# traveller59/spconv

Measured on NVIDIA H100. Metric: active-voxels/sec fwd+bwd SubMConv3d 3^3 C=64, higher is better.
Workload: dtype fp16

## Files before the change

spconv_b200/csrc/common.cuh:

```cuda
#pragma once
#include <cuda_runtime.h>
#include <cuda_fp16.h>
#include <cuda_bf16.h>
#include <stdint.h>
#include <stdio.h>
#include <string.h>
#include <stdarg.h>
#include <type_traits>

#include "../../include/spconv_b200.h"

namespace spx {

void set_error(const char *fmt, ...);
void count_launch(int n = 1);
void set_family(int f);
int sm_count();
int current_device();

struct RuntimeCfg {
    int force_simt = 0, force_tc = 0;
    int debug = 0;
    long long *trace = nullptr;
};
// ... 61 lines not shown
template <typename T> __device__ __forceinline__ float to_float(T v);
template <> __device__ __forceinline__ float to_float<float>(float v) { return v; }
template <> __device__ __forceinline__ float to_float<__half>(__half v) { return __half2float(v); }
template <> __device__ __forceinline__ float to_float<__nv_bfloat16>(__nv_bfloat16 v) { return __bfloat162float(v); }
template <> __device__ __forceinline__ float to_float<int8_t>(int8_t v) { return (float)v; }

template <typename T> __device__ __forceinline__ T from_float(float v);
template <> __device__ __forceinline__ float from_float<float>(float v) { return v; }
template <> __device__ __forceinline__ __half from_float<__half>(float v) { return __float2half_rn(v); }
template <> __device__ __forceinline__ __nv_bfloat16 from_float<__nv_bfloat16>(float v) { return __float2bfloat16_rn(v); }

__device__ __forceinline__ float apply_act(float v, int act, float alpha) {
    switch (act) {
        case SPX_ACT_RELU: return v > 0.f ? v : 0.f;
        case SPX_ACT_SIGMOID: return 1.f / (1.f + __expf(-v));
        case SPX_ACT_LEAKY_RELU: return v >= 0.f ? v : v * alpha;
        default: return v;
    }
}

__device__ __forceinline__ uint32_t smem_u32(const void *p) {
    return (uint32_t)__cvta_generic_to_shared(p);
}

__device__ __forceinline__ void mbar_init(uint64_t *bar, uint32_t count) {
    asm volatile("mbarrier.init.shared::cta.b64 [%0], %1;" ::"r"(smem_u32(bar)), "r"(count) : "memory");
}
__device__ __forceinline__ void mbar_fence_init() {
    asm volatile("fence.mbarrier_init.release.cluster;" ::: "memory");
}
__device__ __forceinline__ void mbar_arrive(uint64_t *bar) {
    asm volatile("{\n\t.reg .b64 st;\n\tmbarrier.arrive.shared::cta.b64 st, [%0];\n\t}" ::"r"(smem_u32(bar)) : "memory");
}
__device__ __forceinline__ void mbar_arrive_expect_tx(uint64_t *bar, uint32_t bytes) {
    asm volatile("{\n\t.reg .b64 st;\n\tmbarrier.arrive.expect_tx.shared::cta.b64 st, [%0], %1;\n\t}" ::"r"(smem_u32(bar)), "r"(bytes) : "memory");
}
__device__ __forceinline__ bool mbar_try_wait(uint64_t *bar, uint32_t parity) {
    uint32_t ok;
    asm volatile(
        "{\n\t.reg .pred p;\n\t"
        "mbarrier.try_wait.parity.shared::cta.b64 p, [%1], %2;\n\t"
        "selp.u32 %0, 1, 0, p;\n\t}"
        : "=r"(ok) : "r"(smem_u32(bar)), "r"(parity) : "memory");
    return ok != 0;
}
__device__ __forceinline__ void mbar_wait(uint64_t *bar, uint32_t parity) {
    if (mbar_try_wait(bar, parity)) return;
    const long long t0 = clock64();
    uint32_t spins = 0;
    while (!mbar_try_wait(bar, parity)) {
        if ((++spins & 0x3FFFu) == 0u && clock64() - t0 > 4000000000ll) {
            printf("spconv_b200: mbarrier wait timed out (block %d thread %d bar 0x%x parity %u)\n",
                   (int)blockIdx.x, (int)threadIdx.x, smem_u32(bar), parity);
            __trap();
        }
    }
}
__device__ __forceinline__ void cp_async_mbar_arrive_noinc(uint64_t *bar) {
    asm volatile("cp.async.mbarrier.arrive.noinc.shared::cta.b64 [%0];" ::"r"(smem_u32(bar)) : "memory");
}

__device__ __forceinline__ void cp_async_16(uint32_t dst_smem, const void *src, uint32_t src_bytes) {
    asm volatile("cp.async.cg.shared.global [%0], [%1], 16, %2;" ::"r"(dst_smem), "l"(src), "r"(src_bytes) : "memory");
}
__device__ __forceinline__ void cp_async_commit() { asm volatile("cp.async.commit_group;" ::: "memory"); }
template <int N> __device__ __forceinline__ void cp_async_wait() {
    asm volatile("cp.async.wait_group %0;" ::"n"(N) : "memory");
}

__device__ __forceinline__ void fence_proxy_async_smem() {
    asm volatile("fence.proxy.async.shared::cta;" ::: "memory");
}

__device__ __forceinline__ void tma_load_2d(uint32_t dst_smem, const void *tmap, uint64_t *bar,
                                            int32_t c0, int32_t c1) {
    asm volatile(
        "cp.async.bulk.tensor.2d.shared::cta.global.tile.mbarrier::complete_tx::bytes [%0], [%1, {%3, %4}], [%2];"
        ::"r"(dst_smem), "l"(tmap), "r"(smem_u32(bar)), "r"(c0), "r"(c1) : "memory");
}
__device__ __forceinline__ void bulk_copy_g2s(uint32_t dst_smem, const void *src, uint32_t bytes, uint64_t *bar) {
    asm volatile("cp.async.bulk.shared::cluster.global.mbarrier::complete_tx::bytes [%0], [%1], %2, [%3];"
                 ::"r"(dst_smem), "l"(src), "r"(bytes), "r"(smem_u32(bar)) : "memory");
}
__device__ __forceinline__ void tma_prefetch_desc(const void *tmap) {
    asm volatile("prefetch.tensormap [%0];" ::"l"(tmap) : "memory");
}

enum MmaKind { KIND_F16 = 0, KIND_TF32 = 1, KIND_I8 = 2 };

__device__ __forceinline__ void wgmma_fence() { asm volatile("wgmma.fence.sync.aligned;" ::: "memory"); }
__device__ __forceinline__ void wgmma_commit() { asm volatile("wgmma.commit_group.sync.aligned;" ::: "memory"); }
template <int N> __device__ __forceinline__ void wgmma_wait() {
    asm volatile("wgmma.wait_group.sync.aligned %0;" ::"n"(N) : "memory");
}
template <typename T, int R> __device__ __forceinline__ void fence_regs(T (&d)[R]) {
#pragma unroll
    for (int i = 0; i < R; ++i) {
        if constexpr (sizeof(T) == 4 && std::is_floating_point<T>::value) asm volatile("" : "+f"(d[i])::"memory");
        else asm volatile("" : "+r"(d[i])::"memory");
    }
}

__host__ __device__ __forceinline__ uint64_t gmma_desc_hi(uint32_t lbo_bytes, uint32_t sbo_bytes, uint32_t swizzle_bytes) {
    const uint64_t layout = swizzle_bytes == 128 ? 1ull : (swizzle_bytes == 64 ? 2ull : 3ull);
    return ((uint64_t)((lbo_bytes >> 4) & 0x3FFF) << 16) | ((uint64_t)((sbo_bytes >> 4) & 0x3FFF) << 32) | (layout << 62);
}

__device__ __forceinline__ uint32_t swizzle_offset(uint32_t off, uint32_t swizzle_bytes) {
    uint32_t bits = swizzle_bytes == 128 ? 7u : (swizzle_bytes == 64 ? 3u : 1u);
    return off ^ (((off >> 7) & bits) << 4);
}

#endif

}
```

spconv_b200/csrc/gemm_tc.cu:

```cuda
#include "gemm.cuh"
#include "wgmma.cuh"
#include <cuda.h>
#include <atomic>
#include <mutex>
#include <stdlib.h>

namespace spx {

constexpr int TC_TILE_M = 128;
constexpr int TC_CONS_WARPS = 8;
constexpr int TC_PROD_WARPS = 2;
constexpr int TC_PROD_THREADS = TC_PROD_WARPS * 32;
constexpr int TC_TMA_WARP = TC_CONS_WARPS + TC_PROD_WARPS;
constexpr int TC_SCHED_WARP = TC_TMA_WARP + 1;
constexpr int TC_THREADS = 3 * 128;
constexpr int TC_INFO_DEPTH = 4;
constexpr int TC_INFO_READERS = TC_PROD_WARPS + TC_CONS_WARPS + 1;
constexpr int TC_MAX_STAGES = 8;
constexpr int TC_SMEM_BUDGET = 200 * 1024;

struct TcParams {
    const uint8_t *x;
    int xb;
    int span_b, b_subtiles, b_sub_bytes, b_bytes, b_mn_major, b_kstep16_mn;
// ... 124 lines not shown
    constexpr int SPAN_A = XB < 128 ? XB : 128;
    constexpr int LG_SPAN_A = SPAN_A == 128 ? 7 : (SPAN_A == 64 ? 6 : 5);
    constexpr int A_SUB_BYTES = TC_TILE_M * SPAN_A;
    constexpr int A_SUBTILES = XB / SPAN_A;
    constexpr int Q_A = SPAN_A / 32;
    constexpr int ROWS_PW = TC_TILE_M / TC_PROD_WARPS;
    constexpr int ITERS = ROWS_PW / RPI > 0 ? ROWS_PW / RPI : 1;
    static_assert(ROWS_PW * CPR >= 32, "a producer warp must cover at least one full cp.async instruction");

    extern __shared__ __align__(1024) uint8_t smem_raw[];
    TC_SPAN(0);
    const uint32_t raw_addr = smem_u32(smem_raw);
    const uint32_t pad = (1024u - (raw_addr & 1023u)) & 1023u;
    uint8_t *smem = smem_raw + pad;
    const uint32_t smem_base = raw_addr + pad;

    const uint32_t idx_off = (uint32_t)p.stages * p.stage_bytes;
    uint64_t *bars = reinterpret_cast<uint64_t *>(smem + idx_off + 2u * p.idx_bytes);
    uint64_t *full = bars;
    uint64_t *empty = bars + TC_MAX_STAGES;
    uint64_t *idx_full = bars + 2 * TC_MAX_STAGES;
    uint64_t *idx_empty = bars + 2 * TC_MAX_STAGES + 2;
    uint64_t *info_full = bars + 2 * TC_MAX_STAGES + 4;
    uint64_t *info_empty = bars + 2 * TC_MAX_STAGES + 4 + TC_INFO_DEPTH;
    int32_t *info = reinterpret_cast<int32_t *>(bars + 2 * TC_MAX_STAGES + 4 + 2 * TC_INFO_DEPTH);

    const int warp = threadIdx.x >> 5;
    const int lane = threadIdx.x & 31;
    const int64_t num_tiles = (p.rows + TC_TILE_M - 1) / TC_TILE_M;

    auto read_info = [&](int n, uint32_t (&tm)[4]) -> int {
        const int e = n & (TC_INFO_DEPTH - 1);
        mbar_wait(&info_full[e], (uint32_t)((n / TC_INFO_DEPTH) & 1));
        const volatile int32_t *r = info + e * 8;
        const int tile = r[0];
        tm[0] = (uint32_t)r[1]; tm[1] = (uint32_t)r[2]; tm[2] = (uint32_t)r[3]; tm[3] = (uint32_t)r[4];
        __syncwarp();
        if (lane == 0) mbar_arrive(&info_empty[e]);
        return tile;
    };

    if (threadIdx.x == 0) {
        for (int s = 0; s < p.stages; ++s) {
            mbar_init(&full[s], TC_PROD_THREADS + 1);
            mbar_init(&empty[s], TC_CONS_WARPS);
        }
        for (int a = 0; a < 2; ++a) {
            mbar_init(&idx_full[a], 1);
            mbar_init(&idx_empty[a], TC_PROD_WARPS);
        }
        for (int e = 0; e < TC_INFO_DEPTH; ++e) {
            mbar_init(&info_full[e], 1);
            mbar_init(&info_empty[e], TC_INFO_READERS);
        }
        mbar_fence_init();
        tma_prefetch_desc(&tmap_w);
    }
    __syncthreads();
    TC_SPAN(1);

    if (warp >= TC_CONS_WARPS && warp < TC_TMA_WARP) {
        const int pw = warp - TC_CONS_WARPS;
        const int r0 = lane >> LG_CPR;
        const uint32_t byte_in_row = (uint32_t)(lane & (CPR - 1)) << 4;
        const uint8_t *x_lane = p.x + byte_in_row;
        uint32_t dst_off[ITERS];
#pragma unroll
        for (int itc = 0; itc < ITERS; ++itc) {
            const uint32_t row_in_tile = (uint32_t)(pw * ROWS_PW + r0 + itc * RPI);
            const uint32_t sub = byte_in_row >> LG_SPAN_A;
            const uint32_t within = byte_in_row & (uint32_t)(SPAN_A - 1);
            dst_off[itc] = sub * (uint32_t)A_SUB_BYTES + swizzle_offset((row_in_tile << LG_SPAN_A) + within, SPAN_A);
        }
        int stage = 0; uint32_t phase = 0;
        for (int n = 0;; ++n) {
            uint32_t tm[4];
            if (read_info(n, tm) < 0) break;
            const int buf = n & 1;
            mbar_wait(&idx_full[buf], (uint32_t)((n >> 1) & 1));
            const int32_t *idx_lane = reinterpret_cast<const int32_t *>(smem + idx_off + (size_t)buf * p.idx_bytes) +
                                      pw * ROWS_PW + r0;
            BitIter it(tm);
            int k = it.next();
            int32_t ridx[ITERS];
            if (k >= 0) {
#pragma unroll
                for (int itc = 0; itc < ITERS; ++itc) ridx[itc] = idx_lane[k * 128 + itc * RPI];
            }
            while (k >= 0) {
                mbar_wait(&empty[stage], phase ^ 1u);
                const uint32_t a_stage = smem_base + (uint32_t)stage * p.stage_bytes;
                if (!(p.debug & 1)) {
#pragma unroll
                    for (int itc = 0; itc < ITERS; ++itc)
                        cp_async_16(a_stage + dst_off[itc], x_lane + (int64_t)max(ridx[itc], 0) * XB,
                                    ridx[itc] >= 0 ? 16u : 0u);
                }
                cp_async_mbar_arrive_noinc(&full[stage]);
                k = it.next();
                if (k >= 0) {
#pragma unroll
                    for (int itc = 0; itc < ITERS; ++itc) ridx[itc] = idx_lane[k * 128 + itc * RPI];
                }
                if (++stage == p.stages) { stage = 0; phase ^= 1u; }
            }
            __syncwarp();
            if (lane == 0) mbar_arrive(&idx_empty[buf]);
        }
    } else if (warp == TC_TMA_WARP) {
        int stage = 0; uint32_t phase = 0;
        for (int n = 0;; ++n) {
            uint32_t tm[4];
            if (read_info(n, tm) < 0) break;
            BitIter it(tm);
            for (int k = it.next(); k >= 0; k = it.next()) {
                mbar_wait(&empty[stage], phase ^ 1u);
                const int kw = p.reverse ? p.kv - 1 - k : k;
                const uint32_t b_stage = smem_base + (uint32_t)stage * p.stage_bytes + p.a_stage_bytes;
                if (p.b_transposed) {
                    const int i4s = p.c_in >> 2;
                    const float *wk = p.w + (int64_t)kw * p.c_in;
                    for (int q = lane; q < p.c_out * i4s; q += 32) {
                        const int o = q / i4s, i4 = (q - o * i4s) * 4;
                        const float4 v = __ldg(reinterpret_cast<const float4 *>(wk + (int64_t)o * p.kv * p.c_in + i4));
                        const uint32_t kb = (uint32_t)o * 4u;
                        const uint32_t sub = kb / (uint32_t)p.span_b, within = kb % (uint32_t)p.span_b;
                        const float vv[4] = {v.x, v.y, v.z, v.w};
#pragma unroll
                        for (int t = 0; t < 4; ++t) {
                            const uint32_t off = sub * (uint32_t)p.b_sub_bytes +
                                                 swizzle_offset((uint32_t)(i4 + t) * (uint32_t)p.span_b + within, (uint32_t)p.span_b);
                            asm volatile("st.shared.f32 [%0], %1;" ::"r"(b_stage + off), "f"(vv[t]) : "memory");
                        }
                    }
                    fence_proxy_async_smem();
                    __syncwarp();
                    if (lane == 0) mbar_arrive(&full[stage]);
                } else if (lane == 0) {
                    if (p.debug & 8) {
                        mbar_arrive(&full[stage]);
                    } else {
                        mbar_arrive_expect_tx(&full[stage], (uint32_t)p.b_bytes);
                        for (int sb = 0; sb < p.b_subtiles; ++sb)
                            tma_load_2d(b_stage + sb * p.b_sub_bytes, &tmap_w, &full[stage],
                                        kw * p.w_inner_elems + sb * p.span_b_elems, 0);
                    }
                }
                __syncwarp();
                if (++stage == p.stages) { stage = 0; phase ^= 1u; }
            }
        }
    } else if (warp == TC_SCHED_WARP) {
        const uint32_t blk_bytes = (uint32_t)(p.kv + 1) * 512u;
        for (int n = 0;; ++n) {
            const int b = n & 1, e = n & (TC_INFO_DEPTH - 1);
            mbar_wait(&idx_empty[b], (uint32_t)(((n >> 1) & 1) ^ 1));
            mbar_wait(&info_empty[e], (uint32_t)(((n / TC_INFO_DEPTH) & 1) ^ 1));
            int tile = -1;
            if (lane == 0) {
                const int ticket = atomicAdd(p.sched_state, 1);
                int4 r0 = make_int4(-1, 1, 0, 0), r1 = make_int4(0, 0, 0, 0);
                if ((int64_t)ticket < num_tiles) {
                    const int4 *rp = reinterpret_cast<const int4 *>(p.sched_rec + (int64_t)ticket * TT_REC_INTS);
                    r0 = __ldg(rp); r1 = __ldg(rp + 1);
                }
                tile = r0.x;
                int32_t *dst = info + e * 8;
                dst[0] = r0.x; dst[1] = r0.y; dst[2] = r0.z; dst[3] = r0.w; dst[4] = r1.x;
                if (tile >= 0) {
                    mbar_arrive_expect_tx(&idx_full[b], blk_bytes);
                    bulk_copy_g2s(smem_base + idx_off + (uint32_t)b * p.idx_bytes,
                                  p.tile_table + (int64_t)tile * (p.kv + 1) * 128, blk_bytes, &idx_full[b]);
                }
                mbar_arrive(&info_full[e]);
            }
            tile = __shfl_sync(0xffffffffu, tile, 0);
            if (tile < 0) break;
        }
        if (lane == 0) {
            __threadfence();
            const int done = atomicAdd(p.sched_state + 1, 1);
            if (done == (int)gridDim.x - 1) {
                p.sched_state[0] = 0;
                p.sched_state[1] = 0;
                __threadfence();
            }
        }
        __syncwarp();
    } else if (warp < TC_CONS_WARPS) {
        const int wg = warp >> 2;
        int stage = 0; uint32_t phase = 0;
        const uint64_t a_hi = gmma_desc_hi(16u, 8u * SPAN_A, SPAN_A);
        const uint64_t b_hi = p.b_mn_major ? gmma_desc_hi((uint32_t)p.b_sub_bytes, 8u * p.span_b, p.span_b)
                                           : gmma_desc_hi(16u, 8u * p.span_b, p.span_b);
        const uint32_t b_sub16 = (uint32_t)p.b_sub_bytes >> 4;
        Acc acc[N / 2];
        for (int local = 0;; ++local) {
            uint32_t tm[4];
            const int tile = read_info(local, tm);
            if (tile < 0) break;
#pragma unroll
            for (int i = 0; i < N / 2; ++i) acc[i] = (Acc)0;
            BitIter it(tm);
            for (int k = it.next(); k >= 0; k = it.next()) {
                mbar_wait(&full[stage], phase);
                fence_proxy_async_smem();
                const uint32_t a16 = (smem_base + (uint32_t)stage * p.stage_bytes + (uint32_t)(wg * 64 * SPAN_A)) >> 4;
                const uint32_t b16 = (smem_base + (uint32_t)stage * p.stage_bytes + (uint32_t)p.a_stage_bytes) >> 4;
                if (!(p.debug & 2)) {
                    fence_regs(acc);
                    wgmma_fence();
                    if (!p.b_mn_major) {
#pragma unroll
                        for (int sub = 0; sub < A_SUBTILES; ++sub) {
                            const uint32_t as = a16 + (uint32_t)sub * (uint32_t)(A_SUB_BYTES >> 4);
                            const uint32_t bs = b16 + (uint32_t)sub * b_sub16;
#pragma unroll
                            for (int jr = 0; jr < Q_A; ++jr)
                                mma_step<KIND, N>(acc, a_hi | (uint64_t)((as + 2u * jr) & 0x3FFFu),
                                                  b_hi | (uint64_t)((bs + 2u * jr) & 0x3FFFu), 0, p.ab_bf16);
                        }
                    } else {
#pragma unroll
                        for (int sub = 0; sub < A_SUBTILES; ++sub) {
                            const uint32_t as = a16 + (uint32_t)sub * (uint32_t)(A_SUB_BYTES >> 4);
#pragma unroll
                            for (int jr = 0; jr < Q_A; ++jr) {
                                const uint32_t j = (uint32_t)(sub * Q_A + jr);
                                mma_step<KIND, N>(acc, a_hi | (uint64_t)((as + 2u * jr) & 0x3FFFu),
                                                  b_hi | (uint64_t)((b16 + j * (uint32_t)p.b_kstep16_mn) & 0x3FFFu), 1,
                                                  p.ab_bf16);
                            }
                        }
                    }
                    wgmma_commit();
                    wgmma_wait<0>();
                    fence_regs(acc);
                }
                __syncwarp();
                if (lane == 0) mbar_arrive(&empty[stage]);
                if (++stage == p.stages) { stage = 0; phase ^= 1u; }
            }
            if (p.debug & 4) continue;
            const int64_t r_lo = (int64_t)tile * TC_TILE_M + wg * 64 + (warp & 3) * 16 + (lane >> 2);
            const int64_t r_hi = r_lo + 8;
            int64_t d_lo = -1, d_hi = -1;
            if (r_lo < p.rows) d_lo = p.argsort ? (int64_t)__ldg(p.argsort + r_lo) : r_lo;
            if (r_hi < p.rows) d_hi = p.argsort ? (int64_t)__ldg(p.argsort + r_hi) : r_hi;
            if constexpr (KIND == KIND_F16) {
                if (p.out_dtype == SPX_F16) epilogue_frag<SPX_F16, false, N>(p, acc, d_lo, d_hi, lane);
                else epilogue_frag<SPX_BF16, false, N>(p, acc, d_lo, d_hi, lane);
            } else if constexpr (KIND == KIND_TF32) {
                epilogue_frag<SPX_F32, false, N>(p, acc, d_lo, d_hi, lane);
            } else {
                if (p.out_dtype == SPX_I8) epilogue_frag<SPX_I8, true, N>(p, acc, d_lo, d_hi, lane);
                else if (p.out_dtype == SPX_F32) epilogue_frag<SPX_F32, true, N>(p, acc, d_lo, d_hi, lane);
                else epilogue_frag<SPX_F16, true, N>(p, acc, d_lo, d_hi, lane);
            }
        }
// ... 201 lines not shown
```

spconv_b200/csrc/gemm_tc_wgrad.cu:

```cuda
#include "gemm.cuh"
#include "peer.cuh"
#include "wgmma.cuh"
#include <stdlib.h>

namespace spx {

constexpr int WG_TILE = 128;
constexpr int WG_CONS_WARPS = 8;
constexpr int WG_PROD_WARPS = 2;
constexpr int WG_PROD_THREADS = WG_PROD_WARPS * 32;
constexpr int WG_SCHED_WARP = WG_CONS_WARPS + WG_PROD_WARPS;
constexpr int WG_THREADS = 3 * 128;
constexpr int WG_ACC_COLS = 256;
constexpr int WG_MAX_STAGES = 6;
constexpr int WG_SMEM_BUDGET = 200 * 1024;
constexpr int WG_SMEM_MAX = 224 * 1024;
constexpr int WG_MAX_IDX = 4;

struct WgParams {
    const uint8_t *x; int xb, span_x, lg_span_x, apo, apg, atom_elems;
    const uint8_t *d; int db, span_d, lg_span_d, lg_cpr_d;
    int n, ab_bf16;
    int groups_total, groups_per_pass;
    int stages, a_stage_bytes, b_buf_bytes, idx_bytes, idx_bufs;
    int64_t rows;
    const int32_t *tile_table;
    const uint32_t *tile_mask;
    const int32_t *sched_rec;
    int kv, words, c_in;
    float *partial; int64_t partial_stride;
    long long *dbg_ts;
    int debug;
};

__device__ __forceinline__ int slot_offset(int slot, int kv) {
    if (slot >= kv) return kv;
    return (slot & 1) ? kv - 1 - (slot >> 1) : (slot >> 1);
}

__device__ __forceinline__ uint32_t active_groups(const uint32_t (&tm)[4], const uint32_t *gmask, int ng, int words) {
    uint32_t act = 0;
    if (words == 1) {
        for (int gl = 0; gl < ng; ++gl) act |= (tm[0] & gmask[gl * 4]) ? 1u << gl : 0u;
        return act;
    }
    for (int gl = 0; gl < ng; ++gl) {
        const uint32_t hit = (tm[0] & gmask[gl * 4]) | (tm[1] & gmask[gl * 4 + 1]) | (tm[2] & gmask[gl * 4 + 2]) |
                             (tm[3] & gmask[gl * 4 + 3]);
        if (hit) act |= 1u << gl;
    }
    return act;
}

__device__ __forceinline__ int64_t wg_rec_index(int64_t i, int chunk, int chunks) {
    return i * chunks + ((i & 1) ? (chunks - 1 - chunk) : chunk);
}
__device__ __forceinline__ void wg_load_rec(const int32_t *__restrict__ rec, int64_t r, int64_t &tile, uint32_t (&m)[4]) {
    const int4 a = __ldg(reinterpret_cast<const int4 *>(rec + r * TT_REC_INTS));
    const int b = __ldg(rec + r * TT_REC_INTS + 4);
    tile = a.x; m[0] = (uint32_t)a.y; m[1] = (uint32_t)a.z; m[2] = (uint32_t)a.w; m[3] = (uint32_t)b;
}

__device__ __forceinline__ long long wg_global_ns() {
    long long t;
    asm volatile("mov.u64 %0, %%globaltimer;" : "=l"(t));
    return t;
}
#define WG_SPAN(i) do { if (p.dbg_ts && threadIdx.x == 0) { const int c_ = blockIdx.y * gridDim.x + blockIdx.x; if (c_ < 512) p.dbg_ts[2 * 2048 + c_ * 4 + (i)] = wg_global_ns(); } } while (0)

__device__ __forceinline__ uint32_t pick_word(const uint32_t (&m)[4], int w) {
    return w == 0 ? m[0] : (w == 1 ? m[1] : (w == 2 ? m[2] : m[3]));
}

__device__ __forceinline__ uint32_t kmajor_tf32_off(uint32_t row, uint32_t voxel, uint32_t rows) {
    return (voxel >> 5) * rows * 128u + swizzle_offset(row * 128u + ((voxel & 31u) << 2), 128u);
}
__device__ __forceinline__ void st_shared_f32x4_t(uint32_t base, uint32_t row0, uint32_t voxel, uint32_t rows, float4 v) {
    const float f[4] = {v.x, v.y, v.z, v.w};
#pragma unroll
    for (int t = 0; t < 4; ++t)
        asm volatile("st.shared.f32 [%0], %1;" ::"r"(base + kmajor_tf32_off(row0 + t, voxel, rows)), "f"(f[t]) : "memory");
}

template <int CPA, int CPD, bool TF32 = false>
__global__ void __launch_bounds__(WG_THREADS, 1)
tc_wgrad_kernel(const WgParams p) {
    constexpr int E = TF32 ? 4 : 2;
    constexpr int N = CPD * 16 / E;
    constexpr int G = WG_ACC_COLS / N < 16 ? WG_ACC_COLS / N : 16;
    constexpr int KSTEPS = WG_TILE * E / 32;
    constexpr int LG_CPA = CPA == 2 ? 1 : (CPA == 4 ? 2 : 3);
    constexpr int RPI = 32 / CPA;
    constexpr int LG_CPD = CPD == 2 ? 1 : (CPD == 4 ? 2 : (CPD == 8 ? 3 : (CPD == 16 ? 4 : 5)));
    constexpr int RPI_D = 32 / CPD;
    constexpr int DB = CPD * 16;
    constexpr int SPAN_D = DB < 128 ? DB : 128;
    constexpr int LG_SPAN_D = SPAN_D == 128 ? 7 : (SPAN_D == 64 ? 6 : 5);
    constexpr int SPAN_X = CPA * 16;
    constexpr int LG_SPAN_X = LG_CPA + 4;
    constexpr int ROWS_PW = WG_TILE / WG_PROD_WARPS;
    constexpr int ITERS = ROWS_PW / RPI > 0 ? ROWS_PW / RPI : 1;
    constexpr int ITERS_D = ROWS_PW / RPI_D;
    extern __shared__ __align__(1024) uint8_t smem_raw[];
    WG_SPAN(0);
    const uint32_t raw_addr = smem_u32(smem_raw);
    const uint32_t pad = (1024u - (raw_addr & 1023u)) & 1023u;
    uint8_t *smem = smem_raw + pad;
    const uint32_t smem_base = raw_addr + pad;
    const uint32_t b_base = smem_base;
    const uint32_t a_base = smem_base + 2u * p.b_buf_bytes;
    const uint32_t idx_off = 2u * p.b_buf_bytes + (uint32_t)p.stages * p.a_stage_bytes;
    uint64_t *bars = reinterpret_cast<uint64_t *>(smem + idx_off + (uint32_t)p.idx_bufs * p.idx_bytes);
    uint64_t *full_a = bars;
    uint64_t *empty_a = bars + WG_MAX_STAGES;
    uint64_t *full_b = bars + 2 * WG_MAX_STAGES;
    uint64_t *empty_b = bars + 2 * WG_MAX_STAGES + 2;
    uint64_t *idx_full = bars + 2 * WG_MAX_STAGES + 4;
    uint64_t *idx_empty = bars + 2 * WG_MAX_STAGES + 4 + WG_MAX_IDX;
    uint32_t *gmask = reinterpret_cast<uint32_t *>(bars + 2 * WG_MAX_STAGES + 4 + 2 * WG_MAX_IDX);
    uint32_t *slot_info = gmask + 32 * 4;

    const int warp = threadIdx.x >> 5;
    const int lane = threadIdx.x & 31;
    const int64_t num_tiles = (p.rows + WG_TILE - 1) / WG_TILE;
    const int chunk = blockIdx.x, chunks = gridDim.x;
    const int g_first = blockIdx.y, g_step = gridDim.y;
    const int ng = g_first < p.groups_total ? (p.groups_total - g_first + g_step - 1) / g_step : 0;

    if (threadIdx.x < 32) {
        const int g = g_first + (int)threadIdx.x * g_step;
        uint32_t m[4] = {0, 0, 0, 0};
        if ((int)threadIdx.x < ng) {
            for (int a = g * p.apg; a < (g + 1) * p.apg; ++a) {
                const int k = slot_offset(a / p.apo, p.kv);
                if (k < p.kv) m[k >> 5] |= 1u << (k & 31);
            }
        }
#pragma unroll
        for (int w = 0; w < 4; ++w) gmask[threadIdx.x * 4 + w] = m[w];
    }
    if (threadIdx.x == 0) {
        for (int s = 0; s < p.stages; ++s) { mbar_init(&full_a[s], WG_PROD_THREADS); mbar_init(&empty_a[s], WG_CONS_WARPS); }
        for (int b = 0; b < 2; ++b) { mbar_init(&full_b[b], WG_PROD_THREADS); mbar_init(&empty_b[b], WG_CONS_WARPS); }
        for (int b = 0; b < p.idx_bufs; ++b) { mbar_init(&idx_full[b], 1); mbar_init(&idx_empty[b], WG_PROD_WARPS); }
        mbar_fence_init();
    }
    __syncthreads();
    WG_SPAN(1);

    if (warp >= WG_CONS_WARPS && warp < WG_SCHED_WARP) {
        const int pw = warp - WG_CONS_WARPS;
        int stage = 0; uint32_t phase = 0;
        int64_t nb = 0;
        const int r0 = lane >> LG_CPA;
        const uint32_t chb = (uint32_t)(lane & (CPA - 1)) << 4;
        const uint8_t *x_lane = p.x + chb;
        uint32_t dst_off[ITERS];
#pragma unroll
        for (int itc = 0; itc < ITERS; ++itc)
            dst_off[itc] = swizzle_offset(((uint32_t)(pw * ROWS_PW + r0 + itc * RPI) << LG_SPAN_X) + chb, SPAN_X);
        const int lg_apo = p.apo == 1 ? 0 : (p.apo == 2 ? 1 : 2);
        const int rd0 = lane >> LG_CPD;
        const uint32_t chd = (uint32_t)(lane & (CPD - 1)) << 4;
        const uint8_t *d_lane = p.d + chd;
        const int nring = p.idx_bufs;
        auto issue_b = [&](const int32_t *idx_s) {
            const int bb = (int)(nb & 1);
            mbar_wait(&empty_b[bb], (uint32_t)(((nb >> 1) & 1) ^ 1));
            const uint32_t dstb = b_base + (uint32_t)bb * p.b_buf_bytes;
            const int32_t *rows_s = idx_s + p.kv * 128 + pw * ROWS_PW + rd0;
            int32_t rsrc[ITERS_D];
#pragma unroll
            for (int itc = 0; itc < ITERS_D; ++itc) rsrc[itc] = rows_s[itc * RPI_D];
            if constexpr (TF32) {
#pragma unroll 1
                for (int i0 = 0; i0 < ITERS_D; i0 += 8) {
                    float4 v[8];
#pragma unroll
                    for (int i = 0; i < 8; ++i) {
                        const int32_t r = i0 + i < ITERS_D ? rsrc[i0 + i] : -1;
                        v[i] = r >= 0 ? __ldg(reinterpret_cast<const float4 *>(d_lane + (int64_t)r * DB)) : make_float4(0.f, 0.f, 0.f, 0.f);
                    }
#pragma unroll
                    for (int i = 0; i < 8; ++i)
                        if (i0 + i < ITERS_D)
                            st_shared_f32x4_t(dstb, chd >> 2, (uint32_t)(pw * ROWS_PW + rd0 + (i0 + i) * RPI_D), (uint32_t)N, v[i]);
                }
                fence_proxy_async_smem();
                mbar_arrive(&full_b[bb]);
            } else {
#pragma unroll
                for (int itc = 0; itc < ITERS_D; ++itc) {
                    const uint32_t row_in_tile = (uint32_t)(pw * ROWS_PW + rd0 + itc * RPI_D);
                    const uint32_t off = (chd >> LG_SPAN_D) * (uint32_t)(WG_TILE * SPAN_D) +
                                         swizzle_offset((row_in_tile << LG_SPAN_D) + (chd & (uint32_t)(SPAN_D - 1)), SPAN_D);
                    cp_async_16(dstb + off, d_lane + (int64_t)max(rsrc[itc], 0) * DB, rsrc[itc] >= 0 ? 16u : 0u);
                }
                cp_async_mbar_arrive_noinc(&full_b[bb]);
            }
            ++nb;
        };
        auto idx_block = [&](int b) {
            return reinterpret_cast<const int32_t *>(smem + idx_off + (size_t)b * p.idx_bytes);
        };
        auto read_slot = [&](int slot, uint32_t use, uint32_t (&m)[4]) -> uint32_t {
            mbar_wait(&idx_full[slot], use & 1u);
            const volatile uint32_t *r = slot_info + slot * 8;
            m[0] = r[1]; m[1] = r[2]; m[2] = r[3]; m[3] = r[4];
            return r[0];
        };
        int cur_slot = 0; uint32_t cur_use = 0;
        uint32_t tm[4] = {0, 0, 0, 0}, tm1[4] = {0, 0, 0, 0};
        uint32_t act = 0;
        if (wg_rec_index(0, chunk, chunks) < num_tiles) {
            act = read_slot(0, 0u, tm);
            if (act) issue_b(idx_block(0));
        }
        for (int64_t step = 0; wg_rec_index(step, chunk, chunks) < num_tiles; ++step) {
            const bool has_next = wg_rec_index(step + 1, chunk, chunks) < num_tiles;
            int nxt_slot = cur_slot + 1; uint32_t nxt_use = cur_use;
            if (nxt_slot == nring) { nxt_slot = 0; ++nxt_use; }
            uint32_t act_next = 0;
            bool next_ready = !has_next;
            auto prepare_next = [&]() {
                act_next = read_slot(nxt_slot, nxt_use, tm1);
                if (act_next) issue_b(idx_block(nxt_slot));
                next_ready = true;
            };
            const int32_t *idx_s = idx_block(cur_slot);
            for (uint32_t rem = act; rem; rem &= rem - 1) {
                const int g = g_first + (__ffs(rem) - 1) * g_step;
                mbar_wait(&empty_a[stage], phase ^ 1u);
                const uint32_t a_stage = a_base + (uint32_t)stage * p.a_stage_bytes;
                for (int s = 0; s < p.apg; ++s) {
                    const int a = g * p.apg + s;
                    const int k = slot_offset(a >> lg_apo, p.kv);
                    const int cb = a & (p.apo - 1);
                    const bool active = k < p.kv && ((pick_word(tm, k >> 5) >> (k & 31)) & 1u);
                    const int32_t *idx_k = idx_s + (active ? k : 0) * 128 + pw * ROWS_PW + r0;
                    const uint8_t *x_atom = x_lane + cb * SPAN_X;
                    int32_t ridx[ITERS];
#pragma unroll
                    for (int itc = 0; itc < ITERS; ++itc) ridx[itc] = active ? idx_k[itc * RPI] : -1;
                    if constexpr (TF32) {
#pragma unroll
                        for (int itc = 0; itc < ITERS; ++itc) {
                            float4 v = make_float4(0.f, 0.f, 0.f, 0.f);
                            if (ridx[itc] >= 0) v = __ldg(reinterpret_cast<const float4 *>(x_atom + (int64_t)ridx[itc] * p.xb));
                            st_shared_f32x4_t(a_stage, (uint32_t)(s * 32) + (chb >> 2),
                                              (uint32_t)(pw * ROWS_PW + r0 + itc * RPI), (uint32_t)WG_TILE, v);
                        }
                    } else {
                        const uint32_t atom_base = a_stage + (uint32_t)s * (uint32_t)(WG_TILE * SPAN_X);
#pragma unroll
                        for (int itc = 0; itc < ITERS; ++itc)
                            cp_async_16(atom_base + dst_off[itc], x_atom + (int64_t)max(ridx[itc], 0) * p.xb,
                                        ridx[itc] >= 0 ? 16u : 0u);
                    }
                }
                if constexpr (TF32) {
                    fence_proxy_async_smem();
                    mbar_arrive(&full_a[stage]);
                } else {
                    cp_async_mbar_arrive_noinc(&full_a[stage]);
                }
                if (++stage == p.stages) { stage = 0; phase ^= 1u; }
                if (!next_ready) prepare_next();
            }
            if (!next_ready) prepare_next();
            __syncwarp();
            if (lane == 0) mbar_arrive(&idx_empty[cur_slot]);
#pragma unroll
            for (int w = 0; w < 4; ++w) tm[w] = tm1[w];
            act = act_next;
            cur_slot = nxt_slot; cur_use = nxt_use;
        }
    } else if (warp == WG_SCHED_WARP) {
        const uint32_t blk_bytes = (uint32_t)(p.kv + 1) * 512u;
        const int nring = p.idx_bufs;
        int slot = 0; uint32_t use = 0;
        uint32_t mw[4] = {0, 0, 0, 0};
        int64_t mtile = 0;
        for (int64_t i = 0; wg_rec_index(i, chunk, chunks) < num_tiles; ++i) {
            if ((i & 31) == 0) {
                const int64_t r = wg_rec_index(i + lane, chunk, chunks);
                if (r < num_tiles) wg_load_rec(p.sched_rec, r, mtile, mw);
            }
            uint32_t tm[4];
#pragma unroll
            for (int w = 0; w < 4; ++w) tm[w] = __shfl_sync(0xffffffffu, mw[w], (int)(i & 31));
            const int64_t tile = __shfl_sync(0xffffffffu, mtile, (int)(i & 31));
            const uint32_t act = active_groups(tm, gmask, ng, p.words);
            mbar_wait(&idx_empty[slot], (use & 1u) ^ 1u);
            if (lane == 0) {
                uint32_t *r = slot_info + slot * 8;
                r[0] = act; r[1] = tm[0]; r[2] = tm[1]; r[3] = tm[2]; r[4] = tm[3];
                if (act) {
                    mbar_arrive_expect_tx(&idx_full[slot], blk_bytes);
                    bulk_copy_g2s(smem_base + idx_off + (uint32_t)slot * p.idx_bytes,
                                  p.tile_table + tile * (int64_t)(p.kv + 1) * 128, blk_bytes, &idx_full[slot]);
                } else {
                    mbar_arrive(&idx_full[slot]);
                }
            }
            __syncwarp();
            if (++slot == nring) { slot = 0; ++use; }
        }
    } else if (warp < WG_CONS_WARPS) {
        const int wg = warp >> 2;
        int stage = 0; uint32_t phase = 0;
        int64_t nb = 0;
        uint32_t tm[4] = {0, 0, 0, 0};
        int64_t tile_unused = 0;
        if (wg_rec_index(0, chunk, chunks) < num_tiles)
            wg_load_rec(p.sched_rec, wg_rec_index(0, chunk, chunks), tile_unused, tm);
        const uint64_t a_hi = TF32 ? gmma_desc_hi(16u, 1024u, 128u)
                                   : gmma_desc_hi((uint32_t)(WG_TILE * SPAN_X), 8u * SPAN_X, SPAN_X);
        const uint64_t b_hi = TF32 ? gmma_desc_hi(16u, 1024u, 128u)
                                   : gmma_desc_hi((uint32_t)(WG_TILE * SPAN_D), 8u * SPAN_D, SPAN_D);
        const uint32_t a_wg = TF32 ? (uint32_t)wg * 64u * 128u : (uint32_t)wg * 64u * WG_TILE * E;
        float acc[G][N / 2];
#pragma unroll
        for (int gl = 0; gl < G; ++gl)
#pragma unroll
            for (int i = 0; i < N / 2; ++i) acc[gl][i] = 0.f;
        for (int64_t step = 0; wg_rec_index(step, chunk, chunks) < num_tiles; ++step) {
            const int64_t next = wg_rec_index(step + 1, chunk, chunks);
            uint32_t tm_next[4] = {0, 0, 0, 0};
            if (next < num_tiles) wg_load_rec(p.sched_rec, next, tile_unused, tm_next);
            const uint32_t act = active_groups(tm, gmask, ng, p.words);
            if (act) {
                const int bb = (int)(nb & 1);
                mbar_wait(&full_b[bb], (uint32_t)((nb >> 1) & 1));
                const uint32_t b16 = (b_base + (uint32_t)bb * p.b_buf_bytes) >> 4;
#pragma unroll
                for (int gl = 0; gl < G; ++gl) {
                    if (!((act >> gl) & 1u)) continue;
                    mbar_wait(&full_a[stage], phase);
                    fence_proxy_async_smem();
                    const uint32_t a16 = (a_base + (uint32_t)stage * p.a_stage_bytes + a_wg) >> 4;
                    fence_regs(acc[gl]);
                    wgmma_fence();
#pragma unroll
                    for (int j = 0; j < KSTEPS; ++j) {
                        if constexpr (TF32) {
                            const uint32_t ao = (uint32_t)(j >> 2) * (WG_TILE * 128u / 16u) + (uint32_t)(j & 3) * 2u;
                            const uint32_t bo = (uint32_t)(j >> 2) * (N * 128u / 16u) + (uint32_t)(j & 3) * 2u;
                            Wgmma<N>::tf32(acc[gl], a_hi | (uint64_t)((a16 + ao) & 0x3FFFu),
                                           b_hi | (uint64_t)((b16 + bo) & 0x3FFFu), 1u);
                        } else {
                            const uint64_t a_desc = a_hi | (uint64_t)((a16 + (uint32_t)j * SPAN_X) & 0x3FFFu);
                            const uint64_t b_desc = b_hi | (uint64_t)((b16 + (uint32_t)j * SPAN_D) & 0x3FFFu);
                            if (p.ab_bf16) Wgmma<N>::template bf16<1, 1>(acc[gl], a_desc, b_desc, 1u);
                            else Wgmma<N>::template f16<1, 1>(acc[gl], a_desc, b_desc, 1u);
                        }
                    }
                    wgmma_commit();
                    wgmma_wait<0>();
                    fence_regs(acc[gl]);
                    __syncwarp();
                    if (lane == 0) mbar_arrive(&empty_a[stage]);
                    if (++stage == p.stages) { stage = 0; phase ^= 1u; }
                }
                __syncwarp();
                if (lane == 0) mbar_arrive(&empty_b[bb]);
                ++nb;
            }
#pragma unroll
            for (int w = 0; w < 4; ++w) tm[w] = tm_next[w];
        }
        WG_SPAN(2);
        if (!(p.debug & 16)) {
            float *part = p.partial + (int64_t)chunk * p.partial_stride;
#pragma unroll
            for (int gl = 0; gl < G; ++gl) {
                if (gl >= ng) break;
                const int g = g_first + gl * g_step;
#pragma unroll
                for (int h = 0; h < 2; ++h) {
                    const int L = wg * 64 + (warp & 3) * 16 + (lane >> 2) + 8 * h;
                    const int s = L / p.atom_elems;
                    const int ce = L - s * p.atom_elems;
                    const int a = g * p.apg + s;
                    const int ks = a / p.apo;
                    const int k = slot_offset(ks, p.kv);
                    const int c = (a - ks * p.apo) * p.atom_elems + ce;
                    if (k >= p.kv) continue;
                    float *dst = part + (int64_t)k * p.c_in + c;
#pragma unroll
                    for (int nb8 = 0; nb8 < N / 8; ++nb8)
#pragma unroll
                        for (int j = 0; j < 2; ++j)
                            dst[(int64_t)(nb8 * 8 + 2 * (lane & 3) + j) * p.kv * p.c_in] = acc[gl][nb8 * 4 + 2 * h + j];
                }
            }
        }
    }

    __syncthreads();
    WG_SPAN(3);
}

constexpr int RED_WARPS = 8;
template <typename T>
__global__ void __launch_bounds__(RED_WARPS * 32)
wgrad_reduce_kernel(const float *__restrict__ partial, int64_t stride, int chunks, int64_t total,
                    T *__restrict__ dw) {
    __shared__ float4 acc_s[RED_WARPS][32];
    const int warp = threadIdx.x >> 5, lane = threadIdx.x & 31;
    const int64_t i = ((int64_t)blockIdx.x * 32 + lane) * 4;
    float4 s = make_float4(0.f, 0.f, 0.f, 0.f);
    if (i < total) {
        const int per = (chunks + RED_WARPS - 1) / RED_WARPS;
        const int c0 = warp * per, c1 = min(chunks, c0 + per);
#pragma unroll 4
        for (int c = c0; c < c1; ++c) {
            const float4 v = __ldg(reinterpret_cast<const float4 *>(partial + (int64_t)c * stride + i));
            s.x += v.x; s.y += v.y; s.z += v.z; s.w += v.w;
        }
    }
    acc_s[warp][lane] = s;
    __syncthreads();
    if (warp == 0 && i < total) {
        float4 t = acc_s[0][lane];
#pragma unroll
        for (int w = 1; w < RED_WARPS; ++w) {
            const float4 v = acc_s[w][lane];
            t.x += v.x; t.y += v.y; t.z += v.z; t.w += v.w;
        }
        dw[i] = from_float<T>(t.x); dw[i + 1] = from_float<T>(t.y);
        dw[i + 2] = from_float<T>(t.z); dw[i + 3] = from_float<T>(t.w);
    }
}

static bool wg_span_ok(int bytes) { return bytes == 32 || bytes == 64 || (bytes >= 128 && bytes % 128 == 0); }

struct WgPlan { WgParams p; int passes, chunks; size_t smem; };

static bool make_plan(const WgradArgs &a, WgPlan &pl) {
    if (a.dtype != SPX_F16 && a.dtype != SPX_BF16 && a.dtype != SPX_F32) return false;
    if (!a.tile_table || !a.tile_mask) return false;
    const bool tf32 = a.dtype == SPX_F32;
    const int e = tf32 ? 4 : 2;
    if (a.c_in % 16 || a.c_out % 16 || a.c_in > 256 || a.c_out > 256) return false;
    if (tf32 && (a.c_in % 32 || a.c_out % 32 || a.c_out > 128 || (runtime_cfg().debug & 4096))) return false;
    if (!wg_span_ok(a.c_in * e) || !wg_span_ok(a.c_out * e)) return false;
    WgParams &p = pl.p;
    memset(&p, 0, sizeof(p));
    p.xb = a.c_in * e; p.span_x = p.xb < 128 ? p.xb : 128;
    p.lg_span_x = p.span_x == 128 ? 7 : (p.span_x == 64 ? 6 : 5);
    p.apo = p.xb / p.span_x;
    p.atom_elems = p.span_x / e;
    p.apg = 128 / p.atom_elems;
    p.db = a.c_out * e; p.span_d = p.db < 128 ? p.db : 128;
    p.lg_span_d = p.span_d == 128 ? 7 : (p.span_d == 64 ? 6 : 5);
    if (p.db & (p.db - 1)) return false;
    p.lg_cpr_d = 0;
    while ((1 << p.lg_cpr_d) < (p.db >> 4)) ++p.lg_cpr_d;
    p.n = a.c_out;
    p.ab_bf16 = a.dtype == SPX_BF16;
    const int atoms_total = a.kv * p.apo;
    p.groups_total = (atoms_total + p.apg - 1) / p.apg;
    p.groups_per_pass = WG_ACC_COLS / a.c_out;
    if (p.groups_per_pass > 16) p.groups_per_pass = 16;
    if ((runtime_cfg().debug & 1024) && p.groups_per_pass >= 2) p.groups_per_pass /= 2;
    pl.passes = (p.groups_total + p.groups_per_pass - 1) / p.groups_per_pass;
    p.a_stage_bytes = p.apg * WG_TILE * p.span_x;
    p.b_buf_bytes = WG_TILE * p.db;
    p.idx_bytes = (int)align_up((size_t)(a.kv + 1) * 512, 1024);
    int avail = (tf32 ? WG_SMEM_MAX - 2048 : WG_SMEM_BUDGET) - 2 * p.b_buf_bytes - 2 * p.idx_bytes;
    if (avail < 2 * p.a_stage_bytes) return false;
    p.stages = avail / p.a_stage_bytes;
    if (p.stages > WG_MAX_STAGES) p.stages = WG_MAX_STAGES;
    size_t fixed = 2 * (size_t)p.b_buf_bytes + (size_t)p.stages * p.a_stage_bytes + 1024 + 1024;
    p.idx_bufs = 2;
    while (p.idx_bufs < WG_MAX_IDX && fixed + (size_t)(p.idx_bufs + 1) * p.idx_bytes <= (size_t)WG_SMEM_MAX) ++p.idx_bufs;
    pl.smem = fixed + (size_t)p.idx_bufs * p.idx_bytes;
    int64_t tiles = div_up64(a.n_out, WG_TILE);
    int chunks = sm_count() / pl.passes;
    if (chunks < 1) chunks = 1;
    if (chunks > tiles) chunks = (int)tiles;
    if (chunks < 1) chunks = 1;
    pl.chunks = chunks;
    p.rows = a.n_out; p.tile_table = a.tile_table; p.tile_mask = a.tile_mask;
    p.sched_rec = a.tile_table + tt_blocks_elems(tiles, a.kv);
    p.kv = a.kv; p.words = (a.kv + 31) / 32; p.c_in = a.c_in;
    p.x = (const uint8_t *)a.x; p.d = (const uint8_t *)a.dout;
    p.partial_stride = (int64_t)a.kv * a.c_in * a.c_out;
    return true;
}

bool tc_wgrad_supported(const WgradArgs &a) {
    WgPlan pl;
    return make_plan(a, pl);
}

size_t tc_wgrad_workspace_size(const WgradArgs &a) {
    WgPlan pl;
    if (!make_plan(a, pl)) return 256;
    return (size_t)pl.chunks * pl.p.partial_stride * sizeof(float) + 256;
}

int tc_wgrad(const WgradArgs &a, cudaStream_t stream) {
    WgPlan pl;
    SPX_REQUIRE(make_plan(a, pl), "tc_wgrad: unsupported shape");
    pl.p.partial = (float *)a.workspace;
    pl.p.dbg_ts = runtime_cfg().trace;
    pl.p.debug = runtime_cfg().debug;
    SPX_REQUIRE((size_t)pl.chunks * pl.p.partial_stride * sizeof(float) <= a.workspace_bytes,
                "tc_wgrad: workspace too small");
    SPX_REQUIRE(((uintptr_t)a.workspace & 15u) == 0, "tc_wgrad: workspace must be 16-byte aligned");
    dim3 grid(pl.chunks, pl.passes);
    const int cpa = pl.p.span_x >> 4, cpd = pl.p.db >> 4;
    using KernelFn = void (*)(const WgParams);
    KernelFn fn = nullptr;
    if (a.dtype == SPX_F32) {
        if (cpa == 8 && cpd == 8) fn = tc_wgrad_kernel<8, 8, true>;
        if (cpa == 8 && cpd == 16) fn = tc_wgrad_kernel<8, 16, true>;
        if (cpa == 8 && cpd == 32) fn = tc_wgrad_kernel<8, 32, true>;
    } else {
#define WG_PICK(A, D) if (cpa == A && cpd == D) fn = tc_wgrad_kernel<A, D>;
#define WG_PICK_ROW(A) WG_PICK(A, 2) WG_PICK(A, 4) WG_PICK(A, 8) WG_PICK(A, 16) WG_PICK(A, 32)
        WG_PICK_ROW(2) WG_PICK_ROW(4) WG_PICK_ROW(8)
#undef WG_PICK_ROW
#undef WG_PICK
    }
    SPX_REQUIRE(fn != nullptr, "tc_wgrad: no kernel instance for this channel layout");
    if (!func_configured((const void *)fn, current_device()))
        SPX_CHECK_CUDA(cudaFuncSetAttribute((const void *)fn, cudaFuncAttributeMaxDynamicSharedMemorySize,
                                            WG_SMEM_MAX));
    fn<<<grid, WG_THREADS, pl.smem, stream>>>(pl.p);
    SPX_CHECK_LAUNCH("tc_wgrad_kernel");
    const int64_t total = pl.p.partial_stride;
    if (a.peers)
        return peer_push(pl.p.partial, total, pl.chunks, nullptr, total, a.dtype, a.peers, stream);
    unsigned nblk = (unsigned)div_up64(total, 128);
    if (a.dtype == SPX_F32)
        wgrad_reduce_kernel<float><<<nblk, RED_WARPS * 32, 0, stream>>>(pl.p.partial, total, pl.chunks, total, (float *)a.dw);
    else if (a.dtype == SPX_F16)
        wgrad_reduce_kernel<__half><<<nblk, RED_WARPS * 32, 0, stream>>>(pl.p.partial, total, pl.chunks, total, (__half *)a.dw);
    else
        wgrad_reduce_kernel<__nv_bfloat16><<<nblk, RED_WARPS * 32, 0, stream>>>(pl.p.partial, total, pl.chunks, total, (__nv_bfloat16 *)a.dw);
    SPX_CHECK_LAUNCH("wgrad_reduce_kernel");
    return 0;
}

}
```

Measured before the change: 456.3 million.

## Copy only active kernel-offset index rows into shared memory per tile

```diff
diff --git a/spconv_b200/csrc/common.cuh b/spconv_b200/csrc/common.cuh
--- a/spconv_b200/csrc/common.cuh
+++ b/spconv_b200/csrc/common.cuh
@@ -167,6 +167,23 @@
     asm volatile("cp.async.bulk.shared::cluster.global.mbarrier::complete_tx::bytes [%0], [%1], %2, [%3];"
                  ::"r"(dst_smem), "l"(src), "r"(bytes), "r"(smem_u32(bar)) : "memory");
 }
+__device__ __forceinline__ void bulk_copy_index_rows(uint32_t dst, const int32_t *block, const uint32_t (&m)[4],
+                                                     int lead, uint64_t *bar, int lane) {
+    uint32_t row = lead >= 0 ? 1u : 0u;
+    if (lane == 0) {
+        const uint32_t rows = row + __popc(m[0]) + __popc(m[1]) + __popc(m[2]) + __popc(m[3]);
+        mbar_arrive_expect_tx(bar, rows * 512u);
+        if (lead >= 0) bulk_copy_g2s(dst, block + lead * 128, 512u, bar);
+    }
+    __syncwarp();
+#pragma unroll
+    for (int w = 0; w < 4; ++w) {
+        if ((m[w] >> lane) & 1u)
+            bulk_copy_g2s(dst + (row + __popc(m[w] & ((1u << lane) - 1u))) * 512u, block + (w * 32 + lane) * 128,
+                          512u, bar);
+        row += __popc(m[w]);
+    }
+}
 __device__ __forceinline__ void tma_prefetch_desc(const void *tmap) {
     asm volatile("prefetch.tensormap [%0];" ::"l"(tmap) : "memory");
 }
diff --git a/spconv_b200/csrc/gemm_tc.cu b/spconv_b200/csrc/gemm_tc.cu
--- a/spconv_b200/csrc/gemm_tc.cu
+++ b/spconv_b200/csrc/gemm_tc.cu
@@ -230,10 +230,11 @@
                                       pw * ROWS_PW + r0;
             BitIter it(tm);
             int k = it.next();
+            int j = 0;
             int32_t ridx[ITERS];
             if (k >= 0) {
 #pragma unroll
-                for (int itc = 0; itc < ITERS; ++itc) ridx[itc] = idx_lane[k * 128 + itc * RPI];
+                for (int itc = 0; itc < ITERS; ++itc) ridx[itc] = idx_lane[itc * RPI];
             }
             while (k >= 0) {
                 mbar_wait(&empty[stage], phase ^ 1u);
@@ -247,8 +248,9 @@
                 cp_async_mbar_arrive_noinc(&full[stage]);
                 k = it.next();
                 if (k >= 0) {
-#pragma unroll
-                    for (int itc = 0; itc < ITERS; ++itc) ridx[itc] = idx_lane[k * 128 + itc * RPI];
+                    ++j;
+#pragma unroll
+                    for (int itc = 0; itc < ITERS; ++itc) ridx[itc] = idx_lane[j * 128 + itc * RPI];
                 }
                 if (++stage == p.stages) { stage = 0; phase ^= 1u; }
             }
@@ -299,30 +301,28 @@
             }
         }
     } else if (warp == TC_SCHED_WARP) {
-        const uint32_t blk_bytes = (uint32_t)(p.kv + 1) * 512u;
         for (int n = 0;; ++n) {
             const int b = n & 1, e = n & (TC_INFO_DEPTH - 1);
             mbar_wait(&idx_empty[b], (uint32_t)(((n >> 1) & 1) ^ 1));
             mbar_wait(&info_empty[e], (uint32_t)(((n / TC_INFO_DEPTH) & 1) ^ 1));
-            int tile = -1;
+            int4 r0 = make_int4(-1, 1, 0, 0), r1 = make_int4(0, 0, 0, 0);
             if (lane == 0) {
                 const int ticket = atomicAdd(p.sched_state, 1);
-                int4 r0 = make_int4(-1, 1, 0, 0), r1 = make_int4(0, 0, 0, 0);
                 if ((int64_t)ticket < num_tiles) {
                     const int4 *rp = reinterpret_cast<const int4 *>(p.sched_rec + (int64_t)ticket * TT_REC_INTS);
                     r0 = __ldg(rp); r1 = __ldg(rp + 1);
                 }
-                tile = r0.x;
                 int32_t *dst = info + e * 8;
                 dst[0] = r0.x; dst[1] = r0.y; dst[2] = r0.z; dst[3] = r0.w; dst[4] = r1.x;
-                if (tile >= 0) {
-                    mbar_arrive_expect_tx(&idx_full[b], blk_bytes);
-                    bulk_copy_g2s(smem_base + idx_off + (uint32_t)b * p.idx_bytes,
-                                  p.tile_table + (int64_t)tile * (p.kv + 1) * 128, blk_bytes, &idx_full[b]);
-                }
-                mbar_arrive(&info_full[e]);
-            }
-            tile = __shfl_sync(0xffffffffu, tile, 0);
+            }
+            const int tile = __shfl_sync(0xffffffffu, r0.x, 0);
+            if (tile >= 0) {
+                const uint32_t tm[4] = {(uint32_t)__shfl_sync(0xffffffffu, r0.y, 0), (uint32_t)__shfl_sync(0xffffffffu, r0.z, 0),
+                                        (uint32_t)__shfl_sync(0xffffffffu, r0.w, 0), (uint32_t)__shfl_sync(0xffffffffu, r1.x, 0)};
+                bulk_copy_index_rows(smem_base + idx_off + (uint32_t)b * p.idx_bytes,
+                                     p.tile_table + (int64_t)tile * (p.kv + 1) * 128, tm, -1, &idx_full[b], lane);
+            }
+            if (lane == 0) mbar_arrive(&info_full[e]);
             if (tile < 0) break;
         }
         if (lane == 0) {
diff --git a/spconv_b200/csrc/gemm_tc_wgrad.cu b/spconv_b200/csrc/gemm_tc_wgrad.cu
--- a/spconv_b200/csrc/gemm_tc_wgrad.cu
+++ b/spconv_b200/csrc/gemm_tc_wgrad.cu
@@ -70,6 +70,14 @@
 
 __device__ __forceinline__ uint32_t pick_word(const uint32_t (&m)[4], int w) {
     return w == 0 ? m[0] : (w == 1 ? m[1] : (w == 2 ? m[2] : m[3]));
+}
+__device__ __forceinline__ int mask_rank(const uint32_t (&m)[4], int k) {
+    const int w = k >> 5;
+    int r = __popc(pick_word(m, w) & ((1u << (k & 31)) - 1u));
+    if (w > 0) r += __popc(m[0]);
+    if (w > 1) r += __popc(m[1]);
+    if (w > 2) r += __popc(m[2]);
+    return r;
 }
 
 __device__ __forceinline__ uint32_t kmajor_tf32_off(uint32_t row, uint32_t voxel, uint32_t rows) {
@@ -168,7 +176,7 @@
             const int bb = (int)(nb & 1);
             mbar_wait(&empty_b[bb], (uint32_t)(((nb >> 1) & 1) ^ 1));
             const uint32_t dstb = b_base + (uint32_t)bb * p.b_buf_bytes;
-            const int32_t *rows_s = idx_s + p.kv * 128 + pw * ROWS_PW + rd0;
+            const int32_t *rows_s = idx_s + pw * ROWS_PW + rd0;
             int32_t rsrc[ITERS_D];
 #pragma unroll
             for (int itc = 0; itc < ITERS_D; ++itc) rsrc[itc] = rows_s[itc * RPI_D];
@@ -237,7 +245,7 @@
                     const int k = slot_offset(a >> lg_apo, p.kv);
                     const int cb = a & (p.apo - 1);
                     const bool active = k < p.kv && ((pick_word(tm, k >> 5) >> (k & 31)) & 1u);
-                    const int32_t *idx_k = idx_s + (active ? k : 0) * 128 + pw * ROWS_PW + r0;
+                    const int32_t *idx_k = idx_s + (active ? 1 + mask_rank(tm, k) : 0) * 128 + pw * ROWS_PW + r0;
                     const uint8_t *x_atom = x_lane + cb * SPAN_X;
                     int32_t ridx[ITERS];
 #pragma unroll
@@ -276,7 +284,6 @@
             cur_slot = nxt_slot; cur_use = nxt_use;
         }
     } else if (warp == WG_SCHED_WARP) {
-        const uint32_t blk_bytes = (uint32_t)(p.kv + 1) * 512u;
         const int nring = p.idx_bufs;
         int slot = 0; uint32_t use = 0;
         uint32_t mw[4] = {0, 0, 0, 0};
@@ -291,17 +298,22 @@
             for (int w = 0; w < 4; ++w) tm[w] = __shfl_sync(0xffffffffu, mw[w], (int)(i & 31));
             const int64_t tile = __shfl_sync(0xffffffffu, mtile, (int)(i & 31));
             const uint32_t act = active_groups(tm, gmask, ng, p.words);
+            uint32_t used[4] = {0, 0, 0, 0};
+            for (uint32_t rem = act; rem; rem &= rem - 1) {
+                const int gl = __ffs(rem) - 1;
+#pragma unroll
+                for (int w = 0; w < 4; ++w) used[w] |= tm[w] & gmask[gl * 4 + w];
+            }
             mbar_wait(&idx_empty[slot], (use & 1u) ^ 1u);
             if (lane == 0) {
                 uint32_t *r = slot_info + slot * 8;
-                r[0] = act; r[1] = tm[0]; r[2] = tm[1]; r[3] = tm[2]; r[4] = tm[3];
-                if (act) {
-                    mbar_arrive_expect_tx(&idx_full[slot], blk_bytes);
-                    bulk_copy_g2s(smem_base + idx_off + (uint32_t)slot * p.idx_bytes,
-                                  p.tile_table + tile * (int64_t)(p.kv + 1) * 128, blk_bytes, &idx_full[slot]);
-                } else {
-                    mbar_arrive(&idx_full[slot]);
-                }
+                r[0] = act; r[1] = used[0]; r[2] = used[1]; r[3] = used[2]; r[4] = used[3];
+            }
+            if (act) {
+                bulk_copy_index_rows(smem_base + idx_off + (uint32_t)slot * p.idx_bytes,
+                                     p.tile_table + tile * (int64_t)(p.kv + 1) * 128, used, p.kv, &idx_full[slot], lane);
+            } else if (lane == 0) {
+                mbar_arrive(&idx_full[slot]);
             }
             __syncwarp();
             if (++slot == nring) { slot = 0; ++use; }
@@ -467,7 +479,9 @@
     pl.passes = (p.groups_total + p.groups_per_pass - 1) / p.groups_per_pass;
     p.a_stage_bytes = p.apg * WG_TILE * p.span_x;
     p.b_buf_bytes = WG_TILE * p.db;
-    p.idx_bytes = (int)align_up((size_t)(a.kv + 1) * 512, 1024);
+    int pass_offsets = p.groups_per_pass * (p.apg > p.apo ? p.apg / p.apo : 1);
+    if (pass_offsets > a.kv) pass_offsets = a.kv;
+    p.idx_bytes = (int)align_up((size_t)(pass_offsets + 1) * 512, 1024);
     int avail = (tf32 ? WG_SMEM_MAX - 2048 : WG_SMEM_BUDGET) - 2 * p.b_buf_bytes - 2 * p.idx_bytes;
     if (avail < 2 * p.a_stage_bytes) return false;
     p.stages = avail / p.a_stage_bytes;
```

Result: no change. 457.3 million, median of 6 (+0.2%).
